# PM25/Information-Retrieval-with-Contrastive-Learning

Hardware: AMD Instinct MI355X
Metric: query-doc pairs/sec (train) + queries/sec @ top-k over N docs, 1/2/4/8 GPU (higher is better)
Workload: dtype bf16

## Files before the change

include/irc.h:

```cpp
#ifndef IRC_H_
#define IRC_H_

#include <stdint.h>

#ifdef __cplusplus
extern "C" {
#endif

typedef void* irc_stream_t;

#define IRC_OK 0
#define IRC_E_INVALID 1001
#define IRC_E_WORKSPACE 1002
#define IRC_E_LAUNCH 1003

const char* irc_last_error(void);
int irc_abi_version(void);

int64_t irc_scan_topk_workspace(int64_t Q, int64_t N, int64_t D, int64_t k);
int irc_scan_topk(const void* queries, const void* docs, int64_t Q, int64_t N, int64_t D,
                  int64_t k, int64_t doc_offset, void* workspace, int64_t workspace_bytes,
                  float* out_score, int64_t* out_idx, irc_stream_t stream);

int irc_scan_topk_many(const void* const* queries, int64_t batches, const void* docs, int64_t Q,
// ... 71 lines not shown
                           int64_t K, int64_t batch);
int irc_gemm_ex(int in_dtype, int out_dtype, int a_layout, int b_layout, int epilogue, int64_t M,
                int64_t N, int64_t K, float alpha, const void* A, int64_t lda, int64_t strideA,
                const void* B, int64_t ldb, int64_t strideB, const float* bias, int64_t strideBias,
                const void* R, int64_t ldr, int64_t strideR, void* C, int64_t ldc, int64_t strideC,
                int accumulate, int64_t batch, void* workspace, int64_t workspace_bytes,
                int64_t max_blocks, irc_stream_t stream);
int64_t irc_gemm_workspace_ex(int in_dtype, int out_dtype, int epilogue, int64_t M, int64_t N,
                              int64_t K, int64_t batch, int64_t max_blocks);
int irc_gemm_set_persistent(int mode);
int irc_gemm_set_big_ring(int on);
int irc_gemm_ln(int epilogue, int64_t M, int64_t N, int64_t K, const void* A, int64_t lda,
                const void* B, int64_t ldb, const float* bias, const void* R, int64_t ldr,
                void* C, int64_t ldc, const float* ln_stats, int ln_nt, const float* ln_gamma,
                const float* ln_beta, float ln_eps, int64_t ln_h, const float* fold_colsum,
                float* stats_out, int* stats_nt_out, irc_stream_t stream);
int irc_gemm_set_big_mf16(int on);
int irc_gemm_set_big_dma(int on);
int irc_gemm_big_dma_fits(int64_t M, int64_t N, int64_t K, int64_t lda, int64_t ldb);
int irc_gemm_set_l2_touch(int mode);
int64_t irc_gemm_l2_touch_map(int operand, int64_t tiles_m, int64_t tiles_n, int64_t window,
                              int64_t lines, int64_t nk, int64_t dist, int32_t* count,
                              int32_t* owner, int32_t* sharers);

int irc_gemm_set_pp(int on);

int irc_embed_ln(int dtype, const int64_t* ids, const void* word, const void* pos,
                 const void* type0, const float* gamma, const float* beta, void* y, int64_t rows,
                 int64_t L, int64_t H, float eps, irc_stream_t stream);
int irc_layernorm(int dtype, const void* x, void* y, const float* gamma, const float* beta,
                  int64_t rows, int64_t H, float eps, irc_stream_t stream);
int irc_attention(int dtype, const void* qkv, const int64_t* mask, void* ctx, int64_t B,
                  int64_t L, int64_t H, int64_t heads, irc_stream_t stream);
int irc_qkv_attention(int64_t M, int64_t H, int64_t heads, int64_t L, const void* x, int64_t ldx,
                      const void* wqkv_perm, const float* bias_perm, const int64_t* mask,
                      void* ctx, int64_t ldc, irc_stream_t stream);

int64_t irc_layernorm_bwd_workspace(int64_t rows, int64_t H);
int irc_layernorm_bwd(int dtype, int dy_dtype, const void* dy, const void* x, const float* gamma,
                      void* dx, float* dgamma, float* dbeta, float* partial,
                      int64_t partial_floats, int64_t rows, int64_t H, float eps, int64_t bcast_L,
                      float dy_scale, int accumulate, irc_stream_t stream);
int irc_attention_bwd(int dtype, const void* qkv, const int64_t* mask, const void* ctx,
                      const void* dctx, void* dqkv, int64_t B, int64_t L, int64_t H,
                      int64_t heads, irc_stream_t stream);
int irc_embed_sum(int dtype, const int64_t* ids, const void* word, const void* pos,
// ... 169 lines not shown
```

information-retrieval-with-contrastive-learning_amd/csrc/gemm_pp.h:

```cpp
#pragma once
#include "irc_common.h"

namespace irc {

struct LnArgs {
  const float* st;
  int nt;
  float inv_h, eps;
  const float* gamma;
  const float* beta;
  const float* fold_s;
  float* st_out;
  int nt_out;
};

__device__ __forceinline__ void ln_row_stats(const LnArgs& l, int row, float& mu, float& r) {
  const float2* p = reinterpret_cast<const float2*>(l.st) + (int64_t)row * l.nt;
  float s = 0.f, q = 0.f;
  for (int t = 0; t < l.nt; ++t) {
    const float2 v = p[t];
    s += v.x;
    q += v.y;
  }
  mu = s * l.inv_h;
  const float var = fmaxf(q * l.inv_h - mu * mu, 0.f);
  r = rsqrtf(var + l.eps);
}

namespace gpp {

struct PArgs {
  const unsigned short* A;
  const unsigned short* B;
  void* C;
  const float* bias;
  const void* R;
  float* P;
  int M, N, K, kchunk;
  int64_t lda, ldb, ldc, ldr;
  int64_t sA, sB, sC, sR, sBias;
  float alpha;
  int accumulate;
  int vec_c;
  const uint64_t* thr;
  uint64_t* keys;
  uint32_t* counts;
  int64_t cap;
  int qpad;
  int stride;
  uint32_t idx_base;
  uint64_t* lists;
  int ls;
  const float* sa;
  const float* sb;
  int group_m;
  const unsigned char* sax;
  const unsigned char* sbx;
  int mpad, npad;
  unsigned char* cx;
  LnArgs ln;
  const int32_t* cand;
  const int64_t* cand_off;
  int64_t n_cand;
  int64_t doc_offset;
  float score_scale;
};

int splits_for(int out_f32, int epi, int64_t M, int64_t N, int64_t K, int64_t batch,
               int64_t budget = 256);
int cu_count();
bool qualifies(int la, int lb, int64_t M, int64_t N, int64_t K, const void* A, int64_t lda,
               int64_t sA, const void* B, int64_t ldb, int64_t sB, int64_t batch, int splits);
void run(int out_f32, int la, int lb, int epi, const PArgs& a, int64_t batch, int splits,
         hipStream_t st, int64_t max_grid = 0);
void run_scan(const PArgs& a, hipStream_t st, bool fp8 = false);
void run_pick(const PArgs& a, hipStream_t st, bool fp8 = false);
constexpr int PICK_TILE = 256;
void run_scores_fp8(const PArgs& a, hipStream_t st);
void run_fp8(int epi, const PArgs& a, hipStream_t st);
void run_mx(int epi, const PArgs& a, hipStream_t st);
void run_ln(int epi, const PArgs& a, hipStream_t st);

}
}
```

information-retrieval-with-contrastive-learning_amd/csrc/gemm_pp.hip:

```cpp
#include "gemm_epi.h"
#include "gemm_pp.h"
#include "mx.h"

#include <atomic>
#include <cstdlib>
#include <mutex>

namespace irc {
namespace gpp {
using namespace irc::gemm;

#ifdef IRC_SCAN_STAMPS
__device__ uint64_t pp_stamps[16];
#define PSTAMP(i)                                                              \
  do {                                                                         \
    if (blockIdx.x == 0 && threadIdx.x == 0)                                   \
      *(volatile uint64_t*)&pp_stamps[(i) + (int)(threadIdx.x & 0)] =          \
          __builtin_amdgcn_s_memrealtime();                                    \
  } while (0)
#else
#define PSTAMP(i) \
  do {            \
  } while (0)
#endif

constexpr int BM = 256, BN = 256, BK = 64, NT = 512;
constexpr int BPITCH = 1024 + 64;
constexpr int slot_bytes(bool kmajor) { return kmajor ? 16384 : 16 * BPITCH; }
constexpr int buf_bytes(bool ak, bool bk) { return 2 * slot_bytes(ak) + 2 * slot_bytes(bk); }
constexpr int LDS_BYTES = 2 * buf_bytes(false, false);
constexpr int EP_PITCH = 68;

template <bool KMAJOR>
__device__ __forceinline__ void stage_half(const unsigned short* __restrict__ X, int64_t ld,
                                           int r0, int nrows, int k0, char* img, int wq,
                                           int lane) {
#pragma unroll
  for (int i = 0; i < 4; ++i) {
    const int p = (i * 4 + wq) * 64 + lane;
    if constexpr (KMAJOR) {
      const int row = p >> 3;
      const int c = (p & 7) ^ (row & 7);
      int gr = r0 + row;
      gr = gr < nrows ? gr : nrows - 1;
      glds16(X + (int64_t)gr * ld + k0 + c * 8, img + (i * 4 + wq) * 1024);
    } else {
      const int blk = i * 4 + wq;
      const int a = lane >> 4;
      int gc = r0 + ((lane & 15) ^ (2 * a)) * 8;
      gc = gc + 8 <= nrows ? gc : nrows - 8;
      glds16(X + (int64_t)(k0 + 4 * blk + a) * ld + gc, img + blk * BPITCH);
    }
  }
}

template <bool KMAJOR>
__device__ __forceinline__ bf16x8 frag(const char* img, int row0, int s, int lane) {
  if constexpr (KMAJOR) {
    const int row = row0 + (lane & 15);
    const int c = 4 * s + (lane >> 4);
    return *reinterpret_cast<const bf16x8*>(img + row * 128 + 16 * (c ^ (row & 7)));
  } else {
    const int q = lane >> 4, a = (lane >> 2) & 3, b = lane & 3;
    const int col = row0 + 4 * b;
    const char* p =
        img + (8 * s + 2 * q) * BPITCH + a * 256 + (((col >> 3) ^ (2 * a)) * 16) + (col & 7) * 2;
    const v4s lo = ds_tr16(p);
    const v4s hi = ds_tr16(p + BPITCH);
    const v4s both[2] = {lo, hi};
    return __builtin_bit_cast(bf16x8, both);
  }
}

typedef int v8i32 __attribute__((ext_vector_type(8)));

template <int OA, int OB>
// ... 10 lines not shown
    IRC_MXS(1, 0) IRC_MXS(1, 1) IRC_MXS(1, 2) IRC_MXS(1, 3)
    IRC_MXS(2, 0) IRC_MXS(2, 1) IRC_MXS(2, 2) IRC_MXS(2, 3)
    IRC_MXS(3, 0) IRC_MXS(3, 1) IRC_MXS(3, 2)
#undef IRC_MXS
    default:
      return mfma_mx<3, 3>(a, b, c, sa, sb);
  }
}

constexpr int MX_SC_OFF = 2 * buf_bytes(true, true);
static_assert(MX_SC_OFF + 2 * 2048 <= LDS_BYTES, "MX scale slots");

__device__ __forceinline__ void stage_scales(const PArgs& g, int m0, int n0, int kt, char* sc,
                                             int grp, int wq, int lane) {
  if (wq != 0) return;
  int ln = lane;
  asm volatile("" : "+v"(ln));
  const bool isb = ln >= 32;
  const unsigned char* src = isb ? g.sbx + (int64_t)kt * g.npad * 4 + (n0 >> 8) * 1024
                                 : g.sax + (int64_t)kt * g.mpad * 4 + (m0 >> 8) * 1024;
  glds16(src + grp * 512 + 16 * (ln & 31), sc + grp * 1024);
}

template <bool AK, bool BK_, bool REDERIVE = false>
__device__ __forceinline__ void stage_tile(const PArgs& g, const unsigned short* A,
                                           const unsigned short* B, int m0, int n0, int k0,
                                           char* base, int grp, int wq, int lane) {
  constexpr int SA = slot_bytes(AK), SB = slot_bytes(BK_);
  if constexpr (REDERIVE) {
    asm volatile("" : "+v"(lane));
  }
  stage_half<AK>(A, g.lda, m0 + 128 * grp, g.M, k0, base + grp * SA, wq, lane);
  stage_half<BK_>(B, g.ldb, n0 + 128 * grp, g.N, k0, base + 2 * SA + grp * SB, wq, lane);
}

#define IRC_PP_G1_EARLY 1

template <bool AK, bool BK_, int F8>
__device__ __forceinline__ void mainloop(const PArgs& g, const unsigned short* A,
                                         const unsigned short* B, int m0, int n0, int kbeg,
                                         int nk, char* lds, int pitch, int par, bool staged,
                                         f32x4 (&acc)[8][4], int grp, int wq, int lane, int* pub,
                                         int pub_val) {
  constexpr int SA = slot_bytes(AK), SB = slot_bytes(BK_);
  constexpr bool G1E = IRC_PP_G1_EARLY != 0 && (F8 == 2 || IRC_PP_G1_EARLY == 2);
  constexpr bool RD = F8 == 2 || G1E;
  const int wn = wq;
  const int bh = wn >> 1, bcol = 64 * (wn & 1);
#pragma unroll
  for (int i = 0; i < 8; ++i)
#pragma unroll
    for (int j = 0; j < 4; ++j) acc[i][j] = (f32x4)0.0f;

  if (nk > 0) {
    if (!staged) stage_tile<AK, BK_>(g, A, B, m0, n0, kbeg, lds + par * pitch, grp, wq, lane);
    if constexpr (F8 == 2) stage_scales(g, m0, n0, kbeg / BK, lds + MX_SC_OFF + par * 2048, grp, wq, lane);
    wait_vmcnt<0>();
    wg_barrier();
    if (grp == 1) {
      if (G1E && nk > 1) {
        stage_tile<AK, BK_, RD>(g, A, B, m0, n0, kbeg + BK, lds + (par ^ 1) * pitch, grp, wq, lane);
        if constexpr (F8 == 2)
          stage_scales(g, m0, n0, kbeg / BK + 1, lds + MX_SC_OFF + (par ^ 1) * 2048, grp, wq, lane);
      }
      wg_barrier();
    }
    for (int kt = 0; kt < nk; ++kt) {
      const int cur = (kt + par) & 1;
#ifdef IRC_PP_DIAG_NODMA
      if (kt + 1 < nk && kt < 0) {
#else
      if (kt + 1 < nk && (grp == 0 || !G1E)) {
#endif
        stage_tile<AK, BK_, RD>(g, A, B, m0, n0, kbeg + (kt + 1) * BK, lds + (cur ^ 1) * pitch,
                                grp, wq, lane);
        if constexpr (F8 == 2)
          stage_scales(g, m0, n0, kbeg / BK + kt + 1, lds + MX_SC_OFF + (cur ^ 1) * 2048, grp, wq,
                       lane);
      }
      const char* la = lds + cur * pitch + grp * SA;
      const char* lb = lds + cur * pitch + 2 * SA + bh * SB;
      bf16x8 fa[8][2], fb[4][2];
      uint2 xa;
      uint32_t xb;
      if constexpr (F8 == 2) {
        const int q = lane >> 4;
#pragma unroll
        for (int c = 0; c < 2; ++c) {
#pragma unroll
          for (int j = 0; j < 4; ++j) fb[j][c] = frag<BK_>(lb, bcol + 16 * j, c, lane);
#pragma unroll
          for (int i = 0; i < 8; ++i) fa[i][c] = frag<AK>(la, 16 * i, c, lane);
        }
        const char* sc = lds + MX_SC_OFF + cur * 2048;
        const int rq = (q * 16 + (lane & 15)) * 8;
        xa = *reinterpret_cast<const uint2*>(sc + grp * 1024 + rq);
        xb = *reinterpret_cast<const uint32_t*>(sc + bh * 1024 + 512 + rq + 4 * (wn & 1));
      } else {
#pragma unroll
        for (int s = 0; s < 2; ++s) {
#pragma unroll
          for (int j = 0; j < 4; ++j) fb[j][s] = frag<BK_>(lb, bcol + 16 * j, s, lane);
#pragma unroll
          for (int i = 0; i < 8; ++i) fa[i][s] = frag<AK>(la, 16 * i, s, lane);
        }
      }
      asm volatile("s_waitcnt lgkmcnt(0)" ::: "memory");
      if (grp == 1) wait_vmcnt<0>();
      wg_barrier();
#ifndef IRC_PP_DIAG_NODMA
      if (G1E && grp == 1 && kt + 2 < nk) {
        stage_tile<AK, BK_, RD>(g, A, B, m0, n0, kbeg + (kt + 2) * BK, lds + cur * pitch, grp, wq,
                                lane);
        if constexpr (F8 == 2)
          stage_scales(g, m0, n0, kbeg / BK + kt + 2, lds + MX_SC_OFF + cur * 2048, grp, wq, lane);
      }
#endif
      __builtin_amdgcn_s_setprio(1);
      if constexpr (F8 == 2) {
#pragma unroll
        for (int i = 0; i < 8; ++i)
#pragma unroll
          for (int j = 0; j < 4; ++j) {
            const bf16x8 a2[2] = {fa[i][0], fa[i][1]};
            const bf16x8 b2[2] = {fb[j][0], fb[j][1]};
            acc[i][j] = mfma_mx_sel(i & 3, j, __builtin_bit_cast(v8i32, a2),
                                    __builtin_bit_cast(v8i32, b2), acc[i][j],
                                    (int)(i < 4 ? xa.x : xa.y), (int)xb);
          }
      } else if constexpr (F8) {
#pragma unroll
        for (int i = 0; i < 8; ++i)
#pragma unroll
          for (int j = 0; j < 4; ++j) {
            const bf16x8 a2[2] = {fa[i][0], fa[i][1]};
            const bf16x8 b2[2] = {fb[j][0], fb[j][1]};
            acc[i][j] = __builtin_amdgcn_mfma_scale_f32_16x16x128_f8f6f4(
                __builtin_bit_cast(v8i32, a2), __builtin_bit_cast(v8i32, b2), acc[i][j], 0, 0, 0,
                127, 0, 127);
          }
      } else {
#pragma unroll
        for (int s = 0; s < 2; ++s)
#pragma unroll
          for (int i = 0; i < 8; ++i)
#pragma unroll
            for (int j = 0; j < 4; ++j)
              acc[i][j] = __builtin_amdgcn_mfma_f32_16x16x32_bf16(fa[i][s], fb[j][s], acc[i][j],
                                                                  0, 0, 0);
      }
      __builtin_amdgcn_s_setprio(0);
      if (grp == 0) {
        wait_vmcnt<0>();
        if (kt == nk - 1 && pub != nullptr && threadIdx.x == 0) {
          *pub = pub_val;
          asm volatile("s_waitcnt vmcnt(0) lgkmcnt(0)" ::: "memory");
        }
      }
      if (!(grp == 1 && kt == nk - 1)) wg_barrier();
    }
  }
}

template <typename TO, int EPI, int F8, bool LN = false>
__device__ __forceinline__ void epilogue_vec(const PArgs& g, const f32x4 (&acc)[8][4], char* lds,
                                             int m0, int n0, int batch, int grp, int wn, int wave,
                                             int lane, int split = 0) {
  const int rbase0 = m0 + 128 * grp;
  const int cbase = n0 + 64 * wn;
  float* st = reinterpret_cast<float*>(lds) + wave * (32 * EP_PITCH);
  const bool slab = g.P != nullptr;
  if (slab || g.vec_c) {
    const float* bias = g.bias ? g.bias + batch * g.sBias : nullptr;
    float bv[4];
#pragma unroll
    for (int j = 0; j < 4; ++j) {
// ... 652 lines not shown
      if (pre && next < ntiles)
        stage_tile<AK, BK_>(g, g.A, g.B, tile_m(next) * BM, tile_n(next) * BN, 0, lds + PBUF, grp,
                            wq, ln);
    };
    if constexpr (EPI == EPI_SCAN) {
      if (g.lists != nullptr)
        epilogue_scan_lists(g, acc, lds, m0, n0, tn, grp, wq, ln, prestage);
      else
        epilogue_scan(g, acc, lds, m0, n0, tn, grp, wq, ln, prestage);
    } else {
      prestage();
      epilogue_vec<TO, EPI, F8>(g, acc, lds, m0, n0, 0, grp, wq, wave, ln);
    }
    if (next >= ntiles) break;
    tile = next;
    if (!pre) wg_barrier();
  }
  if (dyn && threadIdx.x == 0 && atomicAdd(ctr + 1, 1u) == (uint32_t)G - 1) {
    atomicExch(ctr, 0u);
    atomicExch(ctr + 1, 0u);
  }
}

}

namespace gpp {

template <bool AK, bool BKM, typename TO>
static void launch_epi(int epi, const PArgs& a, dim3 grid, hipStream_t st) {
  switch (epi) {
#define IRC_PP(E)                                                                           \
  case E:                                                                                   \
    hipLaunchKernelGGL((gemm_pp_kernel<AK, BKM, TO, E>), grid, dim3(NT), 0, st, a); \
    break;
    IRC_PP(0) IRC_PP(1) IRC_PP(2) IRC_PP(3) IRC_PP(4) IRC_PP(5) IRC_PP(6)
#undef IRC_PP
  }
}

template <typename TO>
static void launch_layout(int la, int lb, int epi, const PArgs& a, dim3 grid, hipStream_t st);

extern "C" int irc_pp_dbg_stamps(uint64_t* out ) {
#ifdef IRC_SCAN_STAMPS
  if (hipDeviceSynchronize() != hipSuccess) return -1;
  return hipMemcpyFromSymbol(out, HIP_SYMBOL(pp_stamps), sizeof(pp_stamps)) == hipSuccess ? 0 : -1;
// ... 206 lines not shown
  }
  if (pgrid > 0) {
    if (out_f32) {
      if (lb == 0) launch_pers<true, true, float>(epi, a, (unsigned)pgrid, ctr, st);
      else launch_pers<true, false, float>(epi, a, (unsigned)pgrid, ctr, st);
    } else {
      if (lb == 0) launch_pers<true, true, unsigned short>(epi, a, (unsigned)pgrid, ctr, st);
      else launch_pers<true, false, unsigned short>(epi, a, (unsigned)pgrid, ctr, st);
    }
    return;
  }
  const dim3 grid((unsigned)tiles, (unsigned)batch, (unsigned)splits);
  if (splits > 1)
    launch_layout<float>(la, lb, 0, a, grid, st);
  else if (out_f32)
    launch_layout<float>(la, lb, epi, a, grid, st);
  else
    launch_layout<unsigned short>(la, lb, epi, a, grid, st);
}

}
}

extern "C" int irc_gemm_set_persistent(int mode) {
  return irc::gpp::pers_mode().exchange(mode < 0 ? 0 : mode > 3 ? 1 : mode);
}
```

information-retrieval-with-contrastive-learning_amd/irc_amd/_lib.py:

```python
from __future__ import annotations

import ctypes
import os
import threading

_HERE = os.path.dirname(os.path.abspath(__file__))
LIB_PATH = os.path.join(_HERE, "lib", "libirc_hip.so")
LIB_PATH = os.environ.get("IRC_LIB_PATH") or LIB_PATH

_c = ctypes
P = _c.c_void_p
I64 = _c.c_int64
I32 = _c.c_int
U32 = _c.c_uint32
F32 = _c.c_float

SIGNATURES = {
    "irc_last_error": (_c.c_char_p, []),
    "irc_abi_version": (I32, []),
    "irc_scan_topk_workspace": (I64, [I64, I64, I64, I64]),
    "irc_scan_topk": (I32, [P, P, I64, I64, I64, I64, I64, P, I64, P, P, P]),
    "irc_scan_topk_many": (I32, [P, I64, P, I64, I64, I64, I64, I64, P, I64, I64, P, P, P, P]),
    "irc_corpus_pack": (I32, [P, P, I64, I64, P, P, P]),
    "irc_pair_sample": (I32, [P, P, P, P, I64, P, P]),
# ... 26 lines not shown
    "irc_csr_union_emit": (I32, [P, I64, I64, P, P, P, P]),
    "irc_csr_spmv_f64": (I32, [P, P, P, I64, P, P, P, I64, P, P]),
    "irc_topk_f64": (I32, [P, I64, P, P, I64, I64, P, P, P, P]),
    "irc_proto_ce": (I32, [P, P, I64, I64, P, P, P, P]),
    "irc_argmax_bias": (I32, [P, P, I64, I64, P, P, P]),
    "irc_centroid_accumulate": (I32, [P, P, I64, I64, P, P, P]),
    "irc_centroid_finalize": (I32, [P, P, I64, I64, P, P, P]),
    "irc_gemm": (I32, [I32, I32, I32, I32, I32, I64, I64, I64, F32, P, I64, I64, P, I64, I64,
                       P, I64, P, I64, I64, P, I64, I64, I32, I64, P, I64, P]),
    "irc_gemm_workspace": (I64, [I32, I32, I32, I64, I64, I64, I64]),
    "irc_gemm_ex": (I32, [I32, I32, I32, I32, I32, I64, I64, I64, F32, P, I64, I64, P, I64, I64,
                          P, I64, P, I64, I64, P, I64, I64, I32, I64, P, I64, I64, P]),
    "irc_gemm_workspace_ex": (I64, [I32, I32, I32, I64, I64, I64, I64, I64]),
    "irc_gemm_set_persistent": (I32, [I32]),
    "irc_gemm_set_big_ring": (I32, [I32]),
    "irc_gemm_ln": (I32, [I32, I64, I64, I64, P, I64, P, I64, P, P, I64, P, I64, P, I32, P, P, F32,
                          I64, P, P, P, P]),
    "irc_gemm_set_big_mf16": (I32, [I32]),
    "irc_gemm_set_big_dma": (I32, [I32]),
    "irc_gemm_big_dma_fits": (I32, [I64, I64, I64, I64, I64]),
    "irc_gemm_set_l2_touch": (I32, [I32]),
    "irc_gemm_l2_touch_map": (I64, [I32, I64, I64, I64, I64, I64, I64, P, P, P]),
    "irc_gemm_set_pp": (I32, [I32]),
    "irc_scan_set_ppl_min_q": (I32, [I32]),
    "irc_embed_ln": (I32, [I32, P, P, P, P, P, P, P, I64, I64, I64, F32, P]),
    "irc_layernorm": (I32, [I32, P, P, P, P, I64, I64, F32, P]),
    "irc_attention": (I32, [I32, P, P, P, I64, I64, I64, I64, P]),
    "irc_qkv_attention": (I32, [I64, I64, I64, I64, P, I64, P, P, P, P, I64, P]),
    "irc_layernorm_bwd_workspace": (I64, [I64, I64]),
    "irc_layernorm_bwd": (I32, [I32, I32, P, P, P, P, P, P, P, I64, I64, I64, F32, I64, F32, I32,
                                P]),
    "irc_attention_bwd": (I32, [I32, P, P, P, P, P, I64, I64, I64, I64, P]),
    "irc_embed_sum": (I32, [I32, P, P, P, P, P, I64, I64, I64, P]),
    "irc_embed_bwd": (I32, [I32, P, P, P, P, P, P, I64, I64, I64, I64, I64, P]),
    "irc_lstm_fwd": (I32, [I32, P, P, P, P, P, P, I64, I64, I64, I64, P]),
    "irc_lstm_bwd": (I32, [I32, P, P, P, P, P, I64, I64, I64, I64, P]),
    "irc_lstm_mfma_supported": (I32, [I64]),
    "irc_lstm_mfma_save_floats": (I64, [I64, I64, I64, I64, I32]),
    "irc_lstm_pack": (I32, [P, P, P, P, I64, I64, I64, P, P, P, P, P]),
    "irc_lstm_fwd_mfma": (I32, [P, P, P, P, P, P, I64, I64, I64, I64, P]),
    "irc_lstm_bwd_mfma": (I32, [P, P, P, P, P, I64, I64, I64, I64, P]),
    "irc_lstm_hprev": (I32, [P, P, I64, I64, I64, I64, P]),
    "irc_lstm_coop_supported": (I32, [I64]),
    "irc_lstm_coop_sizes": (I64, [I64, I64, I64, I64, I32]),
    "irc_lstm_coop_pack": (I32, [P, I64, I64, P, P, P]),
    "irc_lstm_fwd_coop": (I32, [P, P, P, P, P, P, P, P, I64, I64, I64, I64, P]),
# ... 85 lines not shown
```

information-retrieval-with-contrastive-learning_amd/irc_amd/lstm_head.py:

```python
from __future__ import annotations

import math
import os

import torch
import torch.nn as nn

from . import ops
from ._torch import side_stream
from .precision import compute_dtype

ALIGN = 16


def lstm_param_specs(input_size, hidden, num_layers, bidirectional, output_size):
    specs = []
    dirs = ["", "_reverse"] if bidirectional else [""]
    for l in range(num_layers):
        in_l = input_size if l == 0 else hidden * len(dirs)
        for d in dirs:
            specs += [(f"lstm.weight_ih_l{l}{d}", (4 * hidden, in_l)),
                      (f"lstm.weight_hh_l{l}{d}", (4 * hidden, hidden)),
                      (f"lstm.bias_ih_l{l}{d}", (4 * hidden,)),
                      (f"lstm.bias_hh_l{l}{d}", (4 * hidden,))]
# ... 266 lines not shown
        H, nd = self.hidden, self.ndir
        g = self.flat_grad
        o = self.offsets
        if kind == "coop":
            dg, sync = ops.lstm_bwd_coop(dy, whhT, gsave, csave, B, L, H, nd)
            ops.lstm_coop_fault(sync, B, nd, self.coop_fault)
        else:
            dg = ops.lstm_bwd_mfma(dy, whhT, gsave, csave, B, L, H, nd)
        In = x.shape[1]
        BL = B * L
        ih, hh = o[f"lstm.weight_ih_l{l}"], o[f"lstm.weight_hh_l{l}"]
        bi, bh = o[f"lstm.bias_ih_l{l}"], o[f"lstm.bias_hh_l{l}"]
        if nd == 2:
            assert o[f"lstm.weight_ih_l{l}_reverse"] == ih + 4 * H * In
            assert o[f"lstm.weight_hh_l{l}_reverse"] == hh + 4 * H * H
            assert o[f"lstm.bias_ih_l{l}_reverse"] == bi + 4 * H
            assert o[f"lstm.bias_hh_l{l}_reverse"] == bh + 4 * H
        mb = SPLIT_MAX_BLOCKS
        dx = ops.gemm(dg, wih_c, out_dtype=torch.float32, max_blocks=mb) if l > 0 else None
        cur = torch.cuda.current_stream(dg.device)
        side = side_stream(dg.device, "lstm_wgrad")
        side.wait_stream(cur)
        with torch.cuda.stream(side):
            ops.gemm_strided(dg, x, g[ih:], M=4 * H, N=In, K=BL, batch=nd, lda=nd * 4 * H,
                             sA=4 * H, ldb=x.stride(0), sB=0, ldc=In, sC=4 * H * In,
                             trans_a=True, b_is_nk=False, accumulate=True, max_blocks=mb)
            ops.gemm_strided(dg, hprev, g[hh:], M=4 * H, N=H, K=BL, batch=nd, lda=nd * 4 * H,
                             sA=4 * H, ldb=H, sB=BL * H, ldc=H, sC=4 * H * H, trans_a=True,
                             b_is_nk=False, accumulate=True, max_blocks=mb)
            db = ops.colsum(dg)
            ops.axpby(g[bi:bi + nd * 4 * H], db, out=g[bi:bi + nd * 4 * H])
            ops.axpby(g[bh:bh + nd * 4 * H], db, out=g[bh:bh + nd * 4 * H])
        for t in (dg, x, hprev):
            t.record_stream(side)
        self._wgrad_pending = side
        return dx

    def check_fault(self):
        if self.coop_fault.device.type != "cuda":
            return
        if int(self.coop_fault.item()) != 0:
            self.coop_fault.zero_()
            raise ops.IRCError(
                "LSTM cluster recurrence (irc_lstm_fwd_coop / irc_lstm_bwd_coop) timed out: "
                "its workgroups were not co-resident; the affected outputs were NaN-poisoned")

    def forward(self, features, **kwargs):
        B, L, In = features.shape
        dt = compute_dtype()
        x = features.reshape(B * L, In).to(dt).contiguous()
        for l in range(self.num_layers):
            x, _ = self._layer_fwd(l, x, B, L, dt, save=False)
        wl = self.view("scaling_layer.0.weight")
        bl = self.view("scaling_layer.0.bias")
        xf = x if x.dtype == torch.float32 else x.float()
        y = ops.gemm(xf.contiguous(), wl, bias=bl, epilogue=ops.EPI_BIAS)
        if self.act_kind != 0:
            y = ops.activation(self.act_kind, y)
        return y.view(B, L, -1)
# ... 25 lines not shown
```

information-retrieval-with-contrastive-learning_amd/irc_amd/ops.py:

```python
from __future__ import annotations

import ctypes

import torch

from . import _lib
from ._lib import IRCError
from ._torch import ptr, require_hip, stream_ptr

BF16, F32 = torch.bfloat16, torch.float32
_DT = {BF16: 0, F32: 1}

EPI_NONE, EPI_BIAS, EPI_BIAS_GELU, EPI_BIAS_RESID, EPI_RESID = 0, 1, 2, 3, 4


def _code(t: torch.Tensor) -> int:
    try:
        return _DT[t.dtype]
    except KeyError:
        raise TypeError(f"irc kernels take bf16 or fp32, got {t.dtype}") from None


def gemm_set_big_ring(on) -> int:
    return int(_lib.load().irc_gemm_set_big_ring(1 if on else 0))
# ... 113 lines not shown


def _splitk_ws(a, out, epilogue, M, N, K, batch, max_blocks=0):
    nws = _lib.load().irc_gemm_workspace_ex(_code(a), _code(out), int(epilogue), M, N, K, batch,
                                            int(max_blocks))
    if nws <= 0:
        return None, 0
    return torch.empty((nws,), dtype=torch.uint8, device=a.device), nws


def gemm_strided(a, b, out, *, M, N, K, batch, lda, sA, ldb, sB, ldc, sC, trans_a=False,
                 b_is_nk=True, alpha=1.0, accumulate=False, max_blocks=0):
    require_hip(a, b, out)
    if a.dtype != b.dtype:
        raise TypeError("gemm operands must share a dtype")
    ws, nws = _splitk_ws(a, out, EPI_NONE, M, N, K, batch, max_blocks)
    _lib.call("irc_gemm_ex", _code(a), _code(out), 1 if trans_a else 0, 0 if b_is_nk else 1,
              EPI_NONE, M, N, K, float(alpha), ptr(a), lda, sA, ptr(b), ldb, sB, None, 0, None,
              0, 0, ptr(out), ldc, sC, 1 if accumulate else 0, batch, ptr(ws), nws,
              int(max_blocks), stream_ptr(a.device))
    return out


def embed_ln(ids, word, pos, type0, gamma, beta, eps=1e-12, out=None):
    require_hip(ids, word, pos, type0, gamma, beta, out)
    B, L = ids.shape
    H = word.shape[1]
    y = torch.empty((B * L, H), dtype=word.dtype, device=word.device) if out is None else out
    _lib.call("irc_embed_ln", _code(word), ptr(ids), ptr(word), ptr(pos), ptr(type0), ptr(gamma),
              ptr(beta), ptr(y), B * L, L, H, float(eps), stream_ptr(word.device))
    return y


def layernorm(x, gamma, beta, eps=1e-12, out=None):
    require_hip(x, gamma, beta)
    out = torch.empty_like(x) if out is None else out
    H = x.shape[-1]
    _lib.call("irc_layernorm", _code(x), ptr(x), ptr(out), ptr(gamma), ptr(beta),
              x.numel() // H, H, float(eps), stream_ptr(x.device))
    return out


def attention(qkv, mask, B, L, H, heads, out=None):
    require_hip(qkv, mask, out)
    ctx = torch.empty((B * L, H), dtype=qkv.dtype, device=qkv.device) if out is None else out
    _lib.call("irc_attention", _code(qkv), ptr(qkv), ptr(mask), ptr(ctx), B, L, H, heads,
# ... 516 lines not shown
```

Measured before the change: 34610.

## Fuse LSTM weight-gradient GEMMs and bias colsum into one grouped launch

Replaces the two strided split-K GEMMs (dW_ih, dW_hh) plus the colsum and two axpby calls for the LSTM weight gradient with a single grouped persistent GEMM kernel. All per-direction problems go into one XCD-aware grid, with ragged-K support that zero-fills the last partial K tile. A second kernel then reduces the split-K partials into the gradient buffer and computes the bias gradients. This cuts launch count and tail idling on the side stream, at the cost of a new workspace allocation per call and more complex tiling and K-tail logic.

```diff
diff --git a/include/irc.h b/include/irc.h
--- a/include/irc.h
+++ b/include/irc.h
@@ -117,6 +117,16 @@
 int64_t irc_gemm_l2_touch_map(int operand, int64_t tiles_m, int64_t tiles_n, int64_t window,
                               int64_t lines, int64_t nk, int64_t dist, int32_t* count,
                               int32_t* owner, int32_t* sharers);
+
+int64_t irc_lstm_wgrad_workspace(int64_t H, int64_t In, int64_t BL, int64_t nd,
+                                 int64_t max_blocks);
+int irc_lstm_wgrad(const void* dg, const void* x, int64_t ldx, const void* hprev,
+                   float* flat_grad, int64_t off_wih, int64_t off_whh, int64_t off_bih,
+                   int64_t off_bhh, int64_t H, int64_t In, int64_t BL, int64_t nd,
+                   int64_t max_blocks, void* workspace, int64_t workspace_bytes,
+                   irc_stream_t stream);
+int64_t irc_lstm_wgrad_plan(int64_t H, int64_t In, int64_t BL, int64_t nd, int64_t max_blocks,
+                            int32_t* blocks, int64_t cap, int64_t* problems);
 
 int irc_gemm_set_pp(int on);
 
diff --git a/information-retrieval-with-contrastive-learning_amd/csrc/gemm_pp.h b/information-retrieval-with-contrastive-learning_amd/csrc/gemm_pp.h
--- a/information-retrieval-with-contrastive-learning_amd/csrc/gemm_pp.h
+++ b/information-retrieval-with-contrastive-learning_amd/csrc/gemm_pp.h
@@ -28,6 +28,38 @@
 }
 
 namespace gpp {
+
+struct Problem {
+  const unsigned short* A;
+  const unsigned short* B;
+  float* P;
+  int64_t ldb;
+  int N, kchunk, splits;
+  int run;
+  int first;
+};
+constexpr int MAX_PROBLEMS = 4;
+struct Group {
+  int n;
+  int total;
+  Problem p[MAX_PROBLEMS];
+};
+
+__host__ __device__ inline int xcd_run_index(int lin, int total) {
+  const int q = total / 8, r = total % 8, x = lin % 8;
+  return (x < r ? x * (q + 1) : r * (q + 1) + (x - r) * q) + lin / 8;
+}
+
+__host__ __device__ inline void group_map(const Group& gr, int M, int w, int& prob, int& tile,
+                                          int& split) {
+  prob = 0;
+  for (int i = 1; i < MAX_PROBLEMS; ++i)
+    if (i < gr.n && w >= gr.p[i].first) prob = i;
+  const int tiles = ((M + 255) / 256) * ((gr.p[prob].N + 255) / 256);
+  const int r = w - gr.p[prob].first;
+  tile = r % tiles;
+  split = (r / tiles) * gr.p[prob].run;
+}
 
 struct PArgs {
   const unsigned short* A;
@@ -64,6 +96,7 @@
   int64_t n_cand;
   int64_t doc_offset;
   float score_scale;
+  Group grp;
 };
 
 int splits_for(int out_f32, int epi, int64_t M, int64_t N, int64_t K, int64_t batch,
@@ -80,6 +113,7 @@
 void run_fp8(int epi, const PArgs& a, hipStream_t st);
 void run_mx(int epi, const PArgs& a, hipStream_t st);
 void run_ln(int epi, const PArgs& a, hipStream_t st);
+void run_grouped(const PArgs& a, hipStream_t st);
 
 }
 }
diff --git a/information-retrieval-with-contrastive-learning_amd/csrc/gemm_pp.hip b/information-retrieval-with-contrastive-learning_amd/csrc/gemm_pp.hip
--- a/information-retrieval-with-contrastive-learning_amd/csrc/gemm_pp.hip
+++ b/information-retrieval-with-contrastive-learning_amd/csrc/gemm_pp.hip
@@ -31,10 +31,10 @@
 constexpr int LDS_BYTES = 2 * buf_bytes(false, false);
 constexpr int EP_PITCH = 68;
 
-template <bool KMAJOR>
+template <bool KMAJOR, bool RAG = false>
 __device__ __forceinline__ void stage_half(const unsigned short* __restrict__ X, int64_t ld,
                                            int r0, int nrows, int k0, char* img, int wq,
-                                           int lane) {
+                                           int lane, int kmax = 0) {
 #pragma unroll
   for (int i = 0; i < 4; ++i) {
     const int p = (i * 4 + wq) * 64 + lane;
@@ -49,9 +49,24 @@
       const int a = lane >> 4;
       int gc = r0 + ((lane & 15) ^ (2 * a)) * 8;
       gc = gc + 8 <= nrows ? gc : nrows - 8;
-      glds16(X + (int64_t)(k0 + 4 * blk + a) * ld + gc, img + blk * BPITCH);
-    }
-  }
+      int kr = k0 + 4 * blk + a;
+      if constexpr (RAG) kr = kr < kmax ? kr : kmax - 1;
+      glds16(X + (int64_t)kr * ld + gc, img + blk * BPITCH);
+    }
+  }
+}
+
+__device__ __forceinline__ void zero_tail(char* base, int grp, int wq, int lane, int kv) {
+  constexpr int S = slot_bytes(false);
+#pragma unroll
+  for (int h = 0; h < 2; ++h)
+#pragma unroll
+    for (int i = 0; i < 4; ++i) {
+      const int blk = i * 4 + wq;
+      if (4 * blk + (lane >> 4) >= kv)
+        *reinterpret_cast<f32x4*>(base + (2 * h + grp) * S + blk * BPITCH + lane * 16) = (f32x4)0.0f;
+    }
+  asm volatile("s_waitcnt lgkmcnt(0)" ::: "memory");
 }
 
 template <bool KMAJOR>
@@ -108,7 +123,7 @@
   glds16(src + grp * 512 + 16 * (ln & 31), sc + grp * 1024);
 }
 
-template <bool AK, bool BK_, bool REDERIVE = false>
+template <bool AK, bool BK_, bool REDERIVE = false, bool RAG = false>
 __device__ __forceinline__ void stage_tile(const PArgs& g, const unsigned short* A,
                                            const unsigned short* B, int m0, int n0, int k0,
                                            char* base, int grp, int wq, int lane) {
@@ -116,20 +131,22 @@
   if constexpr (REDERIVE) {
     asm volatile("" : "+v"(lane));
   }
-  stage_half<AK>(A, g.lda, m0 + 128 * grp, g.M, k0, base + grp * SA, wq, lane);
-  stage_half<BK_>(B, g.ldb, n0 + 128 * grp, g.N, k0, base + 2 * SA + grp * SB, wq, lane);
+  stage_half<AK, RAG>(A, g.lda, m0 + 128 * grp, g.M, k0, base + grp * SA, wq, lane, g.K);
+  stage_half<BK_, RAG>(B, g.ldb, n0 + 128 * grp, g.N, k0, base + 2 * SA + grp * SB, wq, lane,
+                       g.K);
 }
 
 #define IRC_PP_G1_EARLY 1
 
-template <bool AK, bool BK_, int F8>
+template <bool AK, bool BK_, int F8, bool RAG = false>
 __device__ __forceinline__ void mainloop(const PArgs& g, const unsigned short* A,
                                          const unsigned short* B, int m0, int n0, int kbeg,
                                          int nk, char* lds, int pitch, int par, bool staged,
                                          f32x4 (&acc)[8][4], int grp, int wq, int lane, int* pub,
-                                         int pub_val) {
+                                         int pub_val, int kv_last = 64) {
   constexpr int SA = slot_bytes(AK), SB = slot_bytes(BK_);
   constexpr bool G1E = IRC_PP_G1_EARLY != 0 && (F8 == 2 || IRC_PP_G1_EARLY == 2);
+  static_assert(!RAG || (!AK && !BK_ && F8 == 0 && !G1E), "ragged K: K-outer bf16 only");
   constexpr bool RD = F8 == 2 || G1E;
   const int wn = wq;
   const int bh = wn >> 1, bcol = 64 * (wn & 1);
@@ -139,9 +156,13 @@
     for (int j = 0; j < 4; ++j) acc[i][j] = (f32x4)0.0f;
 
   if (nk > 0) {
-    if (!staged) stage_tile<AK, BK_>(g, A, B, m0, n0, kbeg, lds + par * pitch, grp, wq, lane);
+    if (!staged)
+      stage_tile<AK, BK_, false, RAG>(g, A, B, m0, n0, kbeg, lds + par * pitch, grp, wq, lane);
     if constexpr (F8 == 2) stage_scales(g, m0, n0, kbeg / BK, lds + MX_SC_OFF + par * 2048, grp, wq, lane);
     wait_vmcnt<0>();
+    if constexpr (RAG) {
+      if (nk == 1 && kv_last < BK) zero_tail(lds + par * pitch, grp, wq, lane, kv_last);
+    }
     wg_barrier();
     if (grp == 1) {
       if (G1E && nk > 1) {
@@ -158,8 +179,8 @@
 #else
       if (kt + 1 < nk && (grp == 0 || !G1E)) {
 #endif
-        stage_tile<AK, BK_, RD>(g, A, B, m0, n0, kbeg + (kt + 1) * BK, lds + (cur ^ 1) * pitch,
-                                grp, wq, lane);
+        stage_tile<AK, BK_, RD, RAG>(g, A, B, m0, n0, kbeg + (kt + 1) * BK,
+                                     lds + (cur ^ 1) * pitch, grp, wq, lane);
         if constexpr (F8 == 2)
           stage_scales(g, m0, n0, kbeg / BK + kt + 1, lds + MX_SC_OFF + (cur ^ 1) * 2048, grp, wq,
                        lane);
@@ -193,6 +214,10 @@
       }
       asm volatile("s_waitcnt lgkmcnt(0)" ::: "memory");
       if (grp == 1) wait_vmcnt<0>();
+      if constexpr (RAG) {
+        if (grp == 1 && kt + 2 == nk && kv_last < BK)
+          zero_tail(lds + (cur ^ 1) * pitch, grp, wq, lane, kv_last);
+      }
       wg_barrier();
 #ifndef IRC_PP_DIAG_NODMA
       if (G1E && grp == 1 && kt + 2 < nk) {
@@ -238,6 +263,10 @@
       __builtin_amdgcn_s_setprio(0);
       if (grp == 0) {
         wait_vmcnt<0>();
+        if constexpr (RAG) {
+          if (kt + 2 == nk && kv_last < BK)
+            zero_tail(lds + (cur ^ 1) * pitch, grp, wq, lane, kv_last);
+        }
         if (kt == nk - 1 && pub != nullptr && threadIdx.x == 0) {
           *pub = pub_val;
           asm volatile("s_waitcnt vmcnt(0) lgkmcnt(0)" ::: "memory");
@@ -936,6 +965,40 @@
   }
 }
 
+template <bool RAG>
+__global__ __launch_bounds__(NT, 1) void gemm_pp_grouped_kernel(PArgs g_in) {
+  __shared__ __attribute__((aligned(1024))) char lds[LDS_BYTES];
+  int prob, tile, s0;
+  group_map(g_in.grp, g_in.M, xcd_run_index((int)blockIdx.x, g_in.grp.total), prob, tile, s0);
+  const Problem& pr = g_in.grp.p[prob];
+  PArgs g = g_in;
+  g.A = pr.A;
+  g.B = pr.B;
+  g.P = pr.P;
+  g.ldb = pr.ldb;
+  g.N = pr.N;
+  g.kchunk = pr.kchunk;
+  const int s1 = min(pr.splits, s0 + pr.run);
+  const int tiles_n = (g.N + BN - 1) / BN;
+  const int m0 = (tile / tiles_n) * BM, n0 = (tile % tiles_n) * BN;
+  const int lane = threadIdx.x & 63;
+  const int wave = __builtin_amdgcn_readfirstlane(threadIdx.x >> 6);
+  const int grp = wave >> 2, wq = wave & 3;
+  f32x4 acc[8][4];
+  for (int s = s0; s < s1; ++s) {
+    int ln = lane;
+    asm volatile("" : "+v"(ln));
+    const int kbeg = s * g.kchunk;
+    const int kend = min(g.K, kbeg + g.kchunk);
+    const int nk = RAG ? (kend - kbeg + BK - 1) / BK : (kend - kbeg) / BK;
+    mainloop<false, false, 0, RAG>(g, g.A, g.B, m0, n0, kbeg, nk, lds, buf_bytes(false, false), 0,
+                                   false, acc, grp, wq, ln, nullptr, 0,
+                                   kend - kbeg - (nk - 1) * BK);
+    epilogue_vec<float, EPI_NONE, 0>(g, acc, lds, m0, n0, 0, grp, wq, wave, ln, s);
+    if (s + 1 < s1) wg_barrier();
+  }
+}
+
 }
 
 namespace gpp {
@@ -1188,6 +1251,285 @@
 }
 }
 
+namespace irc {
+namespace gpp {
+
+void run_grouped(const PArgs& a, hipStream_t st) {
+  const dim3 grid((unsigned)a.grp.total);
+  if (a.K % BK == 0)
+    hipLaunchKernelGGL(gemm_pp_grouped_kernel<false>, grid, dim3(NT), 0, st, a);
+  else
+    hipLaunchKernelGGL(gemm_pp_grouped_kernel<true>, grid, dim3(NT), 0, st, a);
+}
+
+struct WgradPlan {
+  int np;
+  int total;
+  struct {
+    int N, splits, kchunk, run, first;
+    int64_t slab;
+  } p[MAX_PROBLEMS];
+  int64_t ws_floats;
+};
+
+static int hh_slices(int64_t M, int64_t N, int64_t K, int64_t batch, int64_t budget) {
+  const int64_t tiles = ((M + 127) / 128) * ((N + 127) / 128) * batch;
+  int64_t s = (2 * budget + tiles - 1) / tiles;
+  if (s > K / 512) s = K / 512;
+  if (s > 32) s = 32;
+  if (s < 2) return 1;
+  const int64_t chunk = ((K + s - 1) / s + 63) / 64 * 64;
+  return (int)((K + chunk - 1) / chunk);
+}
+
+static bool wgrad_plan(int64_t H, int64_t In, int64_t BL, int64_t nd, int64_t max_blocks,
+                       WgradPlan& w) {
+  if (H < 2 || In < 8 || BL < 1 || nd < 1 || 2 * nd > MAX_PROBLEMS || (4 * H) % 8 || In % 8 ||
+      H % 8 || BL >= (1ll << 31) || In >= (1ll << 24) || H >= (1ll << 22))
+    return false;
+  const int64_t M = 4 * H;
+  const int64_t bud = max_blocks > 0 ? max_blocks : 256;
+  const int64_t tm = (M + 255) / 256;
+  const int s_ih = splits_for(1, 0, M, In, BL, nd, bud);
+  const int s_hh = hh_slices(M, H, BL, nd, bud);
+  const int g_hh = std::min(s_ih, s_hh);
+  w.np = (int)(2 * nd);
+  int first = 0;
+  int64_t slab = 0;
+  for (int i = 0; i < w.np; ++i) {
+    const bool ih = i < nd;
+    const int64_t N = ih ? In : H;
+    int s = ih ? s_ih : s_hh;
+    const int kchunk = s > 1 ? (int)(((BL + s - 1) / s + 63) / 64 * 64) : (int)BL;
+    s = (int)((BL + kchunk - 1) / kchunk);
+    const int run = ih ? 1 : (s + g_hh - 1) / g_hh;
+    w.p[i].N = (int)N;
+    w.p[i].splits = s;
+    w.p[i].kchunk = kchunk;
+    w.p[i].run = run;
+    w.p[i].first = first;
+    w.p[i].slab = slab;
+    const int64_t items = tm * ((N + 255) / 256) * ((s + run - 1) / run);
+    if (first + items >= (1ll << 30)) return false;
+    first += (int)items;
+    slab += (int64_t)s * M * N;
+  }
+  w.total = first;
+  w.ws_floats = slab;
+  return true;
+}
+
+struct WgradReduce {
+  int np;
+  int nbias;
+  int C;
+  struct {
+    const float* P;
+    float* dst;
+    int64_t mn;
+    int64_t first;
+    int S;
+  } p[MAX_PROBLEMS];
+  int64_t items;
+  const unsigned short* dg;
+  int64_t ldg, BL;
+  float* bih;
+  float* bhh;
+};
+
+constexpr int WR_NT = 1024;
+constexpr int WR_ROWS = WR_NT / 8;
+
+__global__ __launch_bounds__(WR_NT) void wgrad_reduce_kernel(WgradReduce g) {
+  __shared__ float red[WR_ROWS][65];
+  const int t = threadIdx.x;
+  if ((int)blockIdx.x < g.nbias) {
+    const int cl = t & 7, rl = t >> 3;
+    const int c8 = 64 * (int)blockIdx.x + 8 * cl;
+    float s[8] = {0.f, 0.f, 0.f, 0.f, 0.f, 0.f, 0.f, 0.f};
+    if (c8 < g.C) {
+      const unsigned short* x = g.dg + c8;
+      int64_t r = rl;
+      for (; r + 15 * WR_ROWS < g.BL; r += 16 * WR_ROWS) {
+        u16x8 v[16];
+#pragma unroll
+        for (int q = 0; q < 16; ++q)
+          v[q] = *reinterpret_cast<const u16x8*>(x + (r + q * WR_ROWS) * g.ldg);
+#pragma unroll
+        for (int q = 0; q < 16; ++q)
+#pragma unroll
+          for (int e = 0; e < 8; ++e) s[e] += bf16_to_f32(v[q][e]);
+      }
+      for (; r < g.BL; r += WR_ROWS) {
+        const u16x8 v = *reinterpret_cast<const u16x8*>(x + r * g.ldg);
+#pragma unroll
+        for (int e = 0; e < 8; ++e) s[e] += bf16_to_f32(v[e]);
+      }
+    }
+#pragma unroll
+    for (int e = 0; e < 8; ++e) red[rl][8 * cl + e] = s[e];
+    __syncthreads();
+    for (int w = WR_ROWS / 2; w >= 1; w >>= 1) {
+      if (rl < w) {
+#pragma unroll
+        for (int e = 0; e < 8; ++e) red[rl][8 * cl + e] += red[rl + w][8 * cl + e];
+      }
+      __syncthreads();
+    }
+    const int c = 64 * (int)blockIdx.x + t;
+    if (t < 64 && c < g.C) {
+      const float db = red[0][t];
+      g.bih[c] += db;
+      g.bhh[c] += db;
+    }
+    return;
+  }
+  const int64_t it = (int64_t)((int)blockIdx.x - g.nbias) * WR_NT + t;
+  if (it >= g.items) return;
+  int pi = 0;
+  for (int i = 1; i < MAX_PROBLEMS; ++i)
+    if (i < g.np && it >= g.p[i].first) pi = i;
+  const int64_t e = (it - g.p[pi].first) * 4;
+  const float* p = g.p[pi].P + e;
+  const int64_t mn = g.p[pi].mn;
+  f32x4 s = (f32x4)0.0f;
+  for (int k = 0; k < g.p[pi].S; ++k) s += *reinterpret_cast<const f32x4*>(p + k * mn);
+  float* dst = g.p[pi].dst + e;
+  if (((uintptr_t)dst & 15) == 0) {
+    *reinterpret_cast<f32x4*>(dst) = *reinterpret_cast<const f32x4*>(dst) + s;
+  } else {
+#pragma unroll
+    for (int q = 0; q < 4; ++q) dst[q] = dst[q] + s[q];
+  }
+}
+
+}
+}
+
+extern "C" int64_t irc_lstm_wgrad_workspace(int64_t H, int64_t In, int64_t BL, int64_t nd,
+                                            int64_t max_blocks) {
+  irc::gpp::WgradPlan w;
+  if (!irc::gpp::wgrad_plan(H, In, BL, nd, max_blocks, w)) return -1;
+  return w.ws_floats * (int64_t)sizeof(float);
+}
+
+extern "C" int64_t irc_lstm_wgrad_plan(int64_t H, int64_t In, int64_t BL, int64_t nd,
+                                       int64_t max_blocks, int32_t* blocks, int64_t cap,
+                                       int64_t* problems) {
+  using namespace irc::gpp;
+  WgradPlan w;
+  if (!wgrad_plan(H, In, BL, nd, max_blocks, w)) return -1;
+  if (problems)
+    for (int i = 0; i < w.np; ++i) {
+      problems[5 * i] = w.p[i].N;
+      problems[5 * i + 1] = w.p[i].splits;
+      problems[5 * i + 2] = w.p[i].kchunk;
+      problems[5 * i + 3] = w.p[i].run;
+      problems[5 * i + 4] = w.p[i].slab;
+    }
+  if (!blocks) return w.total;
+  if (cap < w.total) return -1;
+  Group gr{};
+  gr.n = w.np;
+  gr.total = w.total;
+  for (int i = 0; i < w.np; ++i) {
+    gr.p[i].N = w.p[i].N;
+    gr.p[i].kchunk = w.p[i].kchunk;
+    gr.p[i].splits = w.p[i].splits;
+    gr.p[i].run = w.p[i].run;
+    gr.p[i].first = w.p[i].first;
+  }
+  const int M = (int)(4 * H);
+  for (int b = 0; b < w.total; ++b) {
+    int prob, tile, s0;
+    group_map(gr, M, xcd_run_index(b, gr.total), prob, tile, s0);
+    const Problem& pr = gr.p[prob];
+    const int tiles_n = (pr.N + 255) / 256;
+    const int s1 = std::min(pr.splits, s0 + pr.run);
+    int32_t* o = blocks + 7 * (int64_t)b;
+    o[0] = prob;
+    o[1] = tile / tiles_n;
+    o[2] = tile % tiles_n;
+    o[3] = s0;
+    o[4] = s1;
+    o[5] = (int32_t)((int64_t)s0 * pr.kchunk);
+    o[6] = (int32_t)std::min<int64_t>(BL, (int64_t)s1 * pr.kchunk);
+  }
+  return w.total;
+}
+
+extern "C" int irc_lstm_wgrad(const void* dg, const void* x, int64_t ldx, const void* hprev,
+                              float* flat_grad, int64_t off_wih, int64_t off_whh, int64_t off_bih,
+                              int64_t off_bhh, int64_t H, int64_t In, int64_t BL, int64_t nd,
+                              int64_t max_blocks, void* workspace, int64_t workspace_bytes,
+                              irc_stream_t stream) {
+  using namespace irc;
+  using namespace irc::gpp;
+  WgradPlan w;
+  IRC_REQUIRE(wgrad_plan(H, In, BL, nd, max_blocks, w),
+              "lstm_wgrad: need 4H, H and In multiples of 8, In >= 8, nd 1 or 2");
+  IRC_REQUIRE(dg && x && hprev && flat_grad, "lstm_wgrad: null operand");
+  IRC_REQUIRE(ldx >= In && ldx % 8 == 0 && (uintptr_t)dg % 16 == 0 && (uintptr_t)x % 16 == 0 &&
+                  (uintptr_t)hprev % 16 == 0 && (uintptr_t)flat_grad % 4 == 0,
+              "lstm_wgrad: operand rows must be 16-byte aligned");
+  IRC_REQUIRE(ldx * BL < (1ll << 40), "lstm_wgrad: x too large");
+  IRC_REQUIRE(off_wih >= 0 && off_whh >= 0 && off_bih >= 0 && off_bhh >= 0,
+              "lstm_wgrad: negative gradient offset");
+  IRC_REQUIRE(workspace && (uintptr_t)workspace % 16 == 0 &&
+                  workspace_bytes >= w.ws_floats * (int64_t)sizeof(float),
+              "lstm_wgrad: workspace smaller than irc_lstm_wgrad_workspace");
+  const int64_t M = 4 * H;
+  const unsigned short* dgp = static_cast<const unsigned short*>(dg);
+  float* ws = static_cast<float*>(workspace);
+  hipStream_t st = as_stream(stream);
+  PArgs pa{};
+  pa.M = (int)M;
+  pa.K = (int)BL;
+  pa.lda = nd * M;
+  pa.alpha = 1.f;
+  pa.grp.n = w.np;
+  pa.grp.total = w.total;
+  WgradReduce rd{};
+  rd.np = w.np;
+  int64_t items = 0;
+  for (int i = 0; i < w.np; ++i) {
+    const bool ih = i < nd;
+    const int d = (int)(ih ? i : i - nd);
+    Problem& p = pa.grp.p[i];
+    p.A = dgp + d * M;
+    p.B = ih ? static_cast<const unsigned short*>(x)
+             : static_cast<const unsigned short*>(hprev) + (int64_t)d * BL * H;
+    p.P = ws + w.p[i].slab;
+    p.ldb = ih ? ldx : H;
+    p.N = w.p[i].N;
+    p.kchunk = w.p[i].kchunk;
+    p.splits = w.p[i].splits;
+    p.run = w.p[i].run;
+    p.first = w.p[i].first;
+    const int64_t mn = M * p.N;
+    rd.p[i].P = p.P;
+    rd.p[i].dst = flat_grad + (ih ? off_wih : off_whh) + d * mn;
+    rd.p[i].mn = mn;
+    rd.p[i].first = items;
+    rd.p[i].S = p.splits;
+    items += mn / 4;
+  }
+  rd.items = items;
+  rd.C = (int)(nd * M);
+  rd.nbias = (rd.C + 63) / 64;
+  rd.dg = dgp;
+  rd.ldg = nd * M;
+  rd.BL = BL;
+  rd.bih = flat_grad + off_bih;
+  rd.bhh = flat_grad + off_bhh;
+  prof_begin(st);
+  run_grouped(pa, st);
+  const int64_t nblk = rd.nbias + (items + WR_NT - 1) / WR_NT;
+  hipLaunchKernelGGL(wgrad_reduce_kernel, dim3((unsigned)nblk), dim3(WR_NT), 0, st, rd);
+  prof_end("gemm_bf16", st, 2.0 * M * (In + H) * BL * nd);
+  return check_launch("lstm_wgrad");
+}
+
 extern "C" int irc_gemm_set_persistent(int mode) {
   return irc::gpp::pers_mode().exchange(mode < 0 ? 0 : mode > 3 ? 1 : mode);
 }
diff --git a/information-retrieval-with-contrastive-learning_amd/irc_amd/_lib.py b/information-retrieval-with-contrastive-learning_amd/irc_amd/_lib.py
--- a/information-retrieval-with-contrastive-learning_amd/irc_amd/_lib.py
+++ b/information-retrieval-with-contrastive-learning_amd/irc_amd/_lib.py
@@ -72,6 +72,10 @@
     "irc_gemm_set_l2_touch": (I32, [I32]),
     "irc_gemm_l2_touch_map": (I64, [I32, I64, I64, I64, I64, I64, I64, P, P, P]),
     "irc_gemm_set_pp": (I32, [I32]),
+    "irc_lstm_wgrad_workspace": (I64, [I64, I64, I64, I64, I64]),
+    "irc_lstm_wgrad": (I32, [P, P, I64, P, P, I64, I64, I64, I64, I64, I64, I64, I64, I64, P, I64,
+                             P]),
+    "irc_lstm_wgrad_plan": (I64, [I64, I64, I64, I64, I64, P, I64, P]),
     "irc_scan_set_ppl_min_q": (I32, [I32]),
     "irc_embed_ln": (I32, [I32, P, P, P, P, P, P, P, I64, I64, I64, F32, P]),
     "irc_layernorm": (I32, [I32, P, P, P, P, I64, I64, F32, P]),
diff --git a/information-retrieval-with-contrastive-learning_amd/irc_amd/lstm_head.py b/information-retrieval-with-contrastive-learning_amd/irc_amd/lstm_head.py
--- a/information-retrieval-with-contrastive-learning_amd/irc_amd/lstm_head.py
+++ b/information-retrieval-with-contrastive-learning_amd/irc_amd/lstm_head.py
@@ -312,19 +312,26 @@
         side = side_stream(dg.device, "lstm_wgrad")
         side.wait_stream(cur)
         with torch.cuda.stream(side):
-            ops.gemm_strided(dg, x, g[ih:], M=4 * H, N=In, K=BL, batch=nd, lda=nd * 4 * H,
-                             sA=4 * H, ldb=x.stride(0), sB=0, ldc=In, sC=4 * H * In,
-                             trans_a=True, b_is_nk=False, accumulate=True, max_blocks=mb)
-            ops.gemm_strided(dg, hprev, g[hh:], M=4 * H, N=H, K=BL, batch=nd, lda=nd * 4 * H,
-                             sA=4 * H, ldb=H, sB=BL * H, ldc=H, sC=4 * H * H, trans_a=True,
-                             b_is_nk=False, accumulate=True, max_blocks=mb)
-            db = ops.colsum(dg)
-            ops.axpby(g[bi:bi + nd * 4 * H], db, out=g[bi:bi + nd * 4 * H])
-            ops.axpby(g[bh:bh + nd * 4 * H], db, out=g[bh:bh + nd * 4 * H])
+            if ops.lstm_wgrad_supported(x, H, In):
+                ops.lstm_wgrad(dg, x, hprev, g, ih, hh, bi, bh, H=H, nd=nd, max_blocks=mb)
+            else:
+                self._wgrad_calls(dg, x, hprev, g, ih, hh, bi, bh, In, BL, mb)
         for t in (dg, x, hprev):
             t.record_stream(side)
         self._wgrad_pending = side
         return dx
+
+    def _wgrad_calls(self, dg, x, hprev, g, ih, hh, bi, bh, In, BL, mb):
+        H, nd = self.hidden, self.ndir
+        ops.gemm_strided(dg, x, g[ih:], M=4 * H, N=In, K=BL, batch=nd, lda=nd * 4 * H,
+                         sA=4 * H, ldb=x.stride(0), sB=0, ldc=In, sC=4 * H * In,
+                         trans_a=True, b_is_nk=False, accumulate=True, max_blocks=mb)
+        ops.gemm_strided(dg, hprev, g[hh:], M=4 * H, N=H, K=BL, batch=nd, lda=nd * 4 * H,
+                         sA=4 * H, ldb=H, sB=BL * H, ldc=H, sC=4 * H * H, trans_a=True,
+                         b_is_nk=False, accumulate=True, max_blocks=mb)
+        db = ops.colsum(dg)
+        ops.axpby(g[bi:bi + nd * 4 * H], db, out=g[bi:bi + nd * 4 * H])
+        ops.axpby(g[bh:bh + nd * 4 * H], db, out=g[bh:bh + nd * 4 * H])
 
     def check_fault(self):
         if self.coop_fault.device.type != "cuda":
diff --git a/information-retrieval-with-contrastive-learning_amd/irc_amd/ops.py b/information-retrieval-with-contrastive-learning_amd/irc_amd/ops.py
--- a/information-retrieval-with-contrastive-learning_amd/irc_amd/ops.py
+++ b/information-retrieval-with-contrastive-learning_amd/irc_amd/ops.py
@@ -159,6 +159,50 @@
     return out
 
 
+def lstm_wgrad_supported(x, H, In) -> bool:
+    return (x.dtype == torch.bfloat16 and In >= 8 and In % 8 == 0 and H % 8 == 0
+            and x.stride(1) == 1 and x.stride(0) % 8 == 0 and x.data_ptr() % 16 == 0)
+
+
+def lstm_wgrad(dg, x, hprev, flat_grad, off_wih, off_whh, off_bih, off_bhh, *, H, nd,
+               max_blocks=0):
+    require_hip(dg, x, hprev, flat_grad)
+    BL, In = x.shape
+    if dg.shape != (BL, nd * 4 * H) or not dg.is_contiguous():
+        raise ValueError("lstm_wgrad: dg must be contiguous [BL, nd*4H]")
+    if hprev.shape != (nd, BL, H) or not hprev.is_contiguous():
+        raise ValueError("lstm_wgrad: hprev must be contiguous [nd, BL, H]")
+    if not (dg.dtype == x.dtype == hprev.dtype == torch.bfloat16) or flat_grad.dtype != F32:
+        raise TypeError("lstm_wgrad: bf16 operands and an fp32 gradient buffer")
+    for off, n in ((off_wih, nd * 4 * H * In), (off_whh, nd * 4 * H * H),
+                   (off_bih, nd * 4 * H), (off_bhh, nd * 4 * H)):
+        if off < 0 or off + n > flat_grad.numel():
+            raise ValueError("lstm_wgrad: gradient block outside flat_grad")
+    nws = int(_lib.load().irc_lstm_wgrad_workspace(H, In, BL, nd, int(max_blocks)))
+    if nws < 0:
+        raise ValueError("lstm_wgrad: unsupported sizes")
+    ws = torch.empty((max(nws, 16),), dtype=torch.uint8, device=dg.device)
+    _lib.call("irc_lstm_wgrad", ptr(dg), ptr(x), x.stride(0), ptr(hprev), ptr(flat_grad),
+              int(off_wih), int(off_whh), int(off_bih), int(off_bhh), H, In, BL, nd,
+              int(max_blocks), ptr(ws), nws, stream_ptr(dg.device))
+
+
+def lstm_wgrad_plan(H, In, BL, nd, max_blocks=0):
+    import numpy as np
+
+    lib = _lib.load()
+    problems = np.zeros((2 * nd, 5), dtype=np.int64)
+    n = int(lib.irc_lstm_wgrad_plan(H, In, BL, nd, int(max_blocks), None, 0,
+                                    problems.ctypes.data))
+    if n < 0:
+        raise ValueError("lstm_wgrad_plan: bad arguments")
+    blocks = np.full((n, 7), -1, dtype=np.int32)
+    got = int(lib.irc_lstm_wgrad_plan(H, In, BL, nd, int(max_blocks), blocks.ctypes.data, n,
+                                      problems.ctypes.data))
+    assert got == n
+    return blocks, problems
+
+
 def embed_ln(ids, word, pos, type0, gamma, beta, eps=1e-12, out=None):
     require_hip(ids, word, pos, type0, gamma, beta, out)
     B, L = ids.shape
```

New measurement: 34720, median of 6. No clear change (+0.3%).
